# ucsdmanorlab/PSSR2

Hardware: AMD Instinct MI355X
Metric: HR tiles/sec (512^2 4xSR) train (higher is better)
Workload: dtype bf16

## Files before the change

include/pssr_mi355.h:

```cpp
#ifndef PSSR_MI355_H
#define PSSR_MI355_H

#include <stdint.h>

#ifdef __cplusplus
extern "C" {
#endif

typedef void* pssr_stream_t;

enum { PSSR_F32 = 0, PSSR_BF16 = 1, PSSR_F16 = 2 };

enum {
    PSSR_OK = 0,
    PSSR_ERR_ARG = -1,
    PSSR_ERR_LAUNCH = -2,
    PSSR_ERR_UNSUPPORTED = -3
};

int pssr_abi_version(void);
const char* pssr_last_error(void);

int pssr_pack_conv_weight(const float* w_oihw, void* packed, int cout, int cin, int ks,
                          int ci_begin, int ci_count, int mode, const int32_t* n_perm,
// ... 217 lines not shown
                         int dtype, pssr_stream_t stream);


int pssr_input_plain(const float* x_nchw, void* out, int n, int c, int h, int w, int out_cs, float pre_scale, float pre_shift,
                     int dtype, pssr_stream_t stream);
int pssr_im2col_dil(const void* in, int in_cs, int in_co, int c, const float* scale, const float* shift, void* col, int cp,
                    int n, int h, int w, int dil, int dtype, pssr_stream_t stream);
int pssr_col2im_dil(const void* dcol, int cp, void* out, int out_cs, int out_co, int c, int n, int h, int w, int dil,
                    const void* y, int y_cs, int y_co, const float* scale, const float* shift, const float* mean,
                    const float* invstd, double* stats, int dtype, pssr_stream_t stream);
int pssr_channel_stats_nhwc(const void* x, int cs, int co, int c, int64_t npix, double* stats, int dtype, pssr_stream_t stream);
int pssr_sum_relu(const void* const* ins, const int* in_cs, const int* in_co, int n_in, void* out, int out_cs, int out_co,
                  int64_t npix, int c, int relu, int dtype, pssr_stream_t stream);
int pssr_relu_mask(const void* dout, int do_cs, int do_co, const void* out, int o_cs, int o_co, void* dz, int dz_cs, int dz_co,
                   int64_t npix, int c, int dtype, pssr_stream_t stream);
int pssr_affine_relu(const void* x, int cs, int co, const float* scale, const float* shift, void* out, int out_cs, int out_co,
                     int64_t npix, int c, int dtype, pssr_stream_t stream);
int pssr_maxpool_k(const void* in, int in_cs, int in_co, void* out, int out_cs, int out_co, int n, int h, int w, int c, int k,
                   int dtype, pssr_stream_t stream);
int pssr_maxpool_k_bwd(const void* act, int act_cs, int act_co, const void* dpool, int dp_cs, int dp_co, void* dx, int dx_cs,
                       int dx_co, int n, int h, int w, int c, int k, int dtype, pssr_stream_t stream);
int pssr_bilinear_up(const void* in, int in_cs, int in_co, void* out, int out_cs, int out_co, int n, int hs, int ws, int h, int w,
                     int c, int dtype, pssr_stream_t stream);
int pssr_bilinear_up_bwd(const void* dout, int do_cs, int do_co, void* din, int di_cs, int di_co, int n, int hs, int ws, int h,
                         int w, int c, int dtype, pssr_stream_t stream);

int pssr_input_patchify(const float* x_nchw, void* xpatch, int n, int c, int h, int w, int ps, int pc,
                        float pre_scale, float pre_shift, const float* scale, const float* shift, int dtype,
                        pssr_stream_t stream);
int pssr_dwconv7_pack(const float* w, float* packed, int c, int flip, pssr_stream_t stream);
#define PSSR_DWPACK_BATCH_MAX 48
typedef struct pssr_dwpack_batch {
    const float* w[PSSR_DWPACK_BATCH_MAX];
    float* packed[PSSR_DWPACK_BATCH_MAX];
    int32_t c[PSSR_DWPACK_BATCH_MAX];
    int32_t flip[PSSR_DWPACK_BATCH_MAX];
} pssr_dwpack_batch;
int pssr_dwconv7_pack_batch(const pssr_dwpack_batch* items, int n_items, pssr_stream_t stream);
int pssr_dwconv7(const void* in, int in_cs, int in_co, const float* w_packed, const float* bias, void* out, int out_cs,
                 int out_co, int n, int h, int w, int c, int accumulate, int dtype, pssr_stream_t stream);
int pssr_dwconv7_wgrad(const void* dy, int dy_cs, int dy_co, const void* x, int x_cs, int x_co, float* dw, int n, int h,
                       int w, int c, int dtype, pssr_stream_t stream);
int64_t pssr_dwconv7_wgrad_workspace_bytes(int n, int h, int w, int c);
int pssr_dwconv7_wgrad_ws(const void* dy, int dy_cs, int dy_co, const void* x, int x_cs, int x_co, float* dw, int n, int h,
                          int w, int c, int dtype, void* workspace, int64_t workspace_bytes, pssr_stream_t stream);
int pssr_layernorm2d_fwd(const void* in, int in_cs, int in_co, const float* gamma, const float* beta, float eps, void* out,
                         int out_cs, int out_co, int s2d, int c_pad, int n, int h, int w, int c, float* mean, float* rstd,
                         int dtype, pssr_stream_t stream);
int pssr_layernorm2d_bwd(const void* g, int g_cs, int g_co, int s2d, int c_pad, const void* x, int x_cs, int x_co,
                         const float* gamma, const float* mean, const float* rstd, void* dx, int dx_cs, int dx_co,
                         int accumulate, int n, int h, int w, int c, double* stats, int dtype, pssr_stream_t stream);
int pssr_image_channel_dot(const void* a, int a_cs, int a_co, const void* b, int b_cs, int b_co, int n, int hw, int c,
                           float scale, float* out, int dtype, pssr_stream_t stream);
int64_t pssr_image_channel_dot_workspace_bytes(int n, int hw, int c);
int pssr_image_channel_dot_ws(const void* a, int a_cs, int a_co, const void* b, int b_cs, int b_co, int n, int hw, int c,
                              float scale, float* out, int dtype, void* workspace, int64_t workspace_bytes, pssr_stream_t stream);
int pssr_ese_gate(const float* s_mean, const float* w_fc, const float* b_fc, int n, int c, float* u, float* gate,
                  pssr_stream_t stream);
int pssr_scale_nc(const void* t, int t_cs, int t_co, const float* gate, const float* gamma, const float* add, void* out,
                  int out_cs, int out_co, int n, int hw, int c, int dtype, pssr_stream_t stream);
int pssr_ese_bwd(const float* A, const float* gate, const float* u, const float* gamma, const float* s_mean,
                 const float* w_fc, int n, int c, int hw, float* du, float* dgamma, float* db_fc, float* dw_fc, float* add,
                 pssr_stream_t stream);

int pssr_head_q_gather(const float* q, const float* bias, float* out_nchw, int n, int h, int w,
                       float out_scale, float out_shift, pssr_stream_t stream);

int pssr_head_conv_fwd(const void* act, int act_cs, int act_co, int blk, const float* w_oihw, const float* bias,
                       float* out_nchw, int n, int h, int w, int cin, int cout, float out_scale, float out_shift,
                       int dtype, pssr_stream_t stream);
int pssr_head_conv_dgrad(const float* g_nchw, float g_scale, const float* w_oihw, const void* act, int act_cs, int act_co,
                         void* dact, int d_cs, int d_co, int blk, int n, int h, int w, int cin, int cout, int dtype,
                         pssr_stream_t stream);
int pssr_head_conv_wgrad(const float* g_nchw, float g_scale, const void* act, int act_cs, int act_co, int blk,
                         float* dw_oihw, int n, int h, int w, int cin, int cout, int dtype, pssr_stream_t stream);
int pssr_head_conv_bwd(const float* g_nchw, float g_scale, const float* w_oihw, const void* act, int act_cs, int act_co,
                       void* dact, int d_cs, int d_co, int blk, float* dw_oihw, float* bias_sum, int n, int h, int w, int cin,
                       int cout, int dtype, pssr_stream_t stream);

int pssr_head_conv_bwd_rows(const float* g_nchw, float g_scale, const float* w_oihw, const void* act, int act_cs, int act_co,
                            void* dact, int d_cs, int d_co, int blk, double* dw_rows, double* bias_rows, int n, int h, int w,
                            int cin, int cout, int dtype, pssr_stream_t stream);

int pssr_sliding_tiles_u8(const uint8_t* sheet, float* tiles, int c, int h, int w, int size, int stride, int tile0, int ntile,
                          pssr_stream_t stream);
int pssr_patch_tiles_u8(const uint8_t* tiles, uint8_t* sheet, int c, int n_rows, int n_cols, int size, int overlap, int margin,
                        pssr_stream_t stream);


int64_t pssr_normalize_preds_workspace_bytes(int64_t pixels_per_image);
int pssr_normalize_preds_u8(const uint8_t* hr, const uint8_t* hr_hat, uint8_t* hr_norm, uint8_t* hr_hat_norm, int n_images,
                            int64_t pixels_per_image, float pmin, float pmax, void* workspace, pssr_stream_t stream);
int64_t pssr_normalize_preds_resized_workspace_bytes(int n_images, int H, int W, int h, int w);
int pssr_normalize_preds_resized_u8(const uint8_t* hr, int H, int W, const uint8_t* hr_hat, int h, int w, uint8_t* hr_norm,
                                    uint8_t* hr_hat_norm, int n_images, float pmin, float pmax, void* workspace,
                                    pssr_stream_t stream);

int64_t pssr_image_metrics_workspace_bytes(int n_images, int h, int w);
int pssr_image_metrics_u8(const uint8_t* hr, const uint8_t* hr_hat, double* out, int n_images, int h, int w, void* workspace,
                          pssr_stream_t stream);

#define PSSR_COPY_BATCH_MAX 16
typedef struct pssr_copy_batch {
    float* dst[PSSR_COPY_BATCH_MAX];
    const float* src[PSSR_COPY_BATCH_MAX];
    int64_t n[PSSR_COPY_BATCH_MAX];
} pssr_copy_batch;
int pssr_copy_f32_batch(const pssr_copy_batch* items, int n_items, pssr_stream_t stream);
typedef struct pssr_fold_batch {
    float* dst[PSSR_COPY_BATCH_MAX];
    const double* src[PSSR_COPY_BATCH_MAX];
    int32_t n[PSSR_COPY_BATCH_MAX];
    int32_t accumulate[PSSR_COPY_BATCH_MAX];
} pssr_fold_batch;
int pssr_f64_to_f32_batch(const pssr_fold_batch* items, int n_items, int stripes, pssr_stream_t stream);

#define PSSR_HIST_CLAMP 1
#define PSSR_HIST_ACCUMULATE 2
#define PSSR_HIST_MAX_BINS 8192
int64_t pssr_gradhist_workspace_bytes(int batch, int64_t n, int bins);
int pssr_gradhist_fwd(const float* a0, const float* b0, const float* a1, const float* b1, float* h0, float* h1, float* workspace,
                      int64_t workspace_bytes, int batch, int64_t n, int bins, float lo, float hi, float sigma, int flags,
                      pssr_stream_t stream);
int pssr_gradhist_bwd(const float* xa, const float* xb, const float* g, const float* g_ref, const float* dev_scale, float g_scale,
                      float* dx, int batch, int64_t n, int bins, float lo, float hi, float sigma, int flags, pssr_stream_t stream);
int pssr_crappifier_profiles(const float* lr_hat, const float* lr, const float* ds_hr, float* pred, float* target, int64_t n, int flags,
                             pssr_stream_t stream);
int pssr_subsample_f32(const float* src, float* dst, int64_t planes, int h_in, int w_in, int stride, pssr_stream_t stream);
int pssr_crappifier_loss_combine(const float* pred_hist, const float* target_hist, int64_t m, const float* ssim_loss, float dist_scale,
                                 float* out, pssr_stream_t stream);
int pssr_crappifier_loss_bwd_scalars(const float* parts, const float* grad_out, float* out, pssr_stream_t stream);
int pssr_clamp_f32(const float* x, float* y, int64_t n, float lo, float hi, pssr_stream_t stream);

#define PSSR_PROFILE_BINS 511
int64_t pssr_noise_profile_workspace_bytes(int images, int64_t per_image);
int pssr_noise_profile_f32(const float* a, const uint8_t* b, int32_t* hist, double* sum, int images, int64_t per_image, void* workspace,
                           int64_t workspace_bytes, pssr_stream_t stream);
int pssr_noise_profile_u8(const uint8_t* a, const uint8_t* b, int32_t* hist, double* sum, int images, int64_t per_image, void* workspace,
                          int64_t workspace_bytes, pssr_stream_t stream);
int pssr_noise_profile_loss(const int32_t* pred_hist, const double* pred_sum, const int32_t* target_hist, const double* target_sum,
                            int images, int64_t per_image, int width, double* loss, double* terms, double* mean, pssr_stream_t stream);

#ifdef __cplusplus
}
#endif
#endif
```

pssr2_amd/_lib.py:

```python
from __future__ import annotations

import ctypes as C
import os
from pathlib import Path

_LIB_PATH = Path(__file__).resolve().parent / "libpssr_mi355.so"
_lib = None

F32, BF16, F16 = 0, 1, 2
PRO_NONE, PRO_BN_RELU, PRO_GELU = 0, 1, 2
EPI_STORE, EPI_TAIL, EPI_DGRAD_MASK, EPI_FINAL, EPI_DGRAD_GELU, EPI_HEADQ = 0, 1, 2, 3, 4, 5
FLAG_RELU, FLAG_STATS, FLAG_AFFINE, FLAG_HEADQ, FLAG_SHUF2, FLAG_SOLO = 1, 2, 4, 8, 16, 32

c_void_p, c_int, c_i64, c_float = C.c_void_p, C.c_int, C.c_int64, C.c_float


class ConvDesc(C.Structure):
    _fields_ = [
        ("dtype", C.c_int32), ("n", C.c_int32), ("h", C.c_int32), ("w", C.c_int32),
        ("in0", c_void_p), ("in0_cstride", C.c_int32), ("in0_coff", C.c_int32), ("cin0", C.c_int32), ("taps0", C.c_int32),
        ("w0", c_void_p),
        ("in1", c_void_p), ("in1_cstride", C.c_int32), ("in1_coff", C.c_int32), ("cin1", C.c_int32), ("taps1", C.c_int32),
        ("w1", c_void_p),
        ("prologue", C.c_int32), ("pro_scale", c_void_p), ("pro_shift", c_void_p),
# ... 8 lines not shown
        ("workspace", c_void_p), ("workspace_bytes", C.c_int64),
        ("head_w", c_void_p), ("head_q", c_void_p),
    ]


class WgradDesc(C.Structure):
    _fields_ = [
        ("dtype", C.c_int32), ("n", C.c_int32), ("h", C.c_int32), ("w", C.c_int32),
        ("dy", c_void_p), ("dy_cstride", C.c_int32), ("dy_coff", C.c_int32), ("dy_blk", C.c_int32), ("cout", C.c_int32),
        ("in_", c_void_p), ("in_cstride", C.c_int32), ("in_coff", C.c_int32), ("in_blk", C.c_int32), ("cin_pad", C.c_int32),
        ("taps", C.c_int32),
        ("prologue", C.c_int32), ("pro_scale", c_void_p), ("pro_shift", c_void_p),
        ("dw", c_void_p), ("dw_parts", C.c_int32),
    ]


class GatherItem(C.Structure):
    _fields_ = [("src", C.c_void_p), ("sh", C.c_int), ("sw", C.c_int), ("rot", C.c_int), ("flip_axis", C.c_int)]


class SheetDesc(C.Structure):
    _fields_ = [("base", C.c_void_p), ("frames", C.c_int), ("h", C.c_int), ("w", C.c_int), ("reserved", C.c_int)]


class WindowItem(C.Structure):
    _fields_ = [("sheet", C.c_int), ("frame0", C.c_int), ("y0", C.c_int), ("x0", C.c_int), ("rot", C.c_int), ("flip_axis", C.c_int)]


class CollagePanel(C.Structure):
    _fields_ = [("src", C.c_void_p), ("image_stride", C.c_int64), ("row_pitch", C.c_int32), ("src_h", C.c_int32), ("src_w", C.c_int32),
                ("is_f32", C.c_int32), ("yi", C.c_void_p), ("xi", C.c_void_p)]


COPY_BATCH_MAX = 16


class FoldBatch(C.Structure):
    _fields_ = [("dst", C.c_void_p * 16), ("src", C.c_void_p * 16), ("n", C.c_int32 * 16), ("accumulate", C.c_int32 * 16)]


DWPACK_BATCH_MAX = 48


class DwPackBatch(C.Structure):
    _fields_ = [("w", C.c_void_p * DWPACK_BATCH_MAX), ("packed", C.c_void_p * DWPACK_BATCH_MAX), ("c", C.c_int32 * DWPACK_BATCH_MAX),
                ("flip", C.c_int32 * DWPACK_BATCH_MAX)]


class CopyBatch(C.Structure):
    _fields_ = [("dst", C.c_void_p * COPY_BATCH_MAX), ("src", C.c_void_p * COPY_BATCH_MAX), ("n", C.c_int64 * COPY_BATCH_MAX)]


class PackItem(C.Structure):
    _fields_ = [("w", c_void_p), ("packed", c_void_p), ("n_perm", c_void_p),
                ("cout", C.c_int32), ("cin", C.c_int32), ("ks", C.c_int32), ("ci_begin", C.c_int32), ("ci_count", C.c_int32),
                ("mode", C.c_int32), ("k_pad", C.c_int32), ("n_pad", C.c_int32), ("dtype", C.c_int32), ("center", C.c_int32)]


def lib():
    global _lib
    if _lib is None:
        if not _LIB_PATH.exists():
            raise RuntimeError(
                f"{_LIB_PATH} not found: build the HIP extension first (python -c 'import __graft_entry__ as g; g.build()' "
                "or make -C pssr2_amd/csrc). pssr2_amd has no CPU fallback.")
        import torch
        _lib = C.CDLL(str(_LIB_PATH))
        _lib.pssr_last_error.restype = C.c_char_p
        _lib.pssr_packed_weight_bytes.restype = C.c_int64
        _lib.pssr_conv2d_workspace_bytes.restype = C.c_int64
        _lib.pssr_gradhist_workspace_bytes.restype = C.c_int64
        _lib.pssr_noise_profile_workspace_bytes.restype = C.c_int64
        _lib.pssr_noise_profile_workspace_bytes.argtypes = [c_int, c_i64]
        for name in ("pssr_noise_profile_f32", "pssr_noise_profile_u8"):
            getattr(_lib, name).argtypes = [c_void_p, c_void_p, c_void_p, c_void_p, c_int, c_i64, c_void_p, c_i64, c_void_p]
        _lib.pssr_noise_profile_loss.argtypes = [c_void_p, c_void_p, c_void_p, c_void_p, c_int, c_i64, c_int, c_void_p, c_void_p, c_void_p,
                                                 c_void_p]
        _lib.pssr_gather_windows_u8.argtypes = [c_void_p, c_int, c_void_p, c_int, c_void_p, c_int, c_int, c_void_p]
        _lib.pssr_collage_rows_u8.argtypes = [c_void_p, c_int, c_void_p, c_i64, c_int, c_int, c_int, c_int, c_void_p]
        _lib.pssr_window_attn_workspace_bytes.restype = c_i64
        _lib.pssr_window_attn_workspace_bytes.argtypes = [c_int] * 5
        _lib.pssr_window_attn_fwd.argtypes = [c_void_p] * 4 + [c_int] * 7 + [c_float, c_int, c_void_p]
        _lib.pssr_window_attn_bwd.argtypes = [c_void_p] * 7 + [c_i64] + [c_int] * 7 + [c_float, c_int, c_void_p]
    return _lib


def check(status: int, what: str):
    if status != 0:
        raise RuntimeError(f"{what} failed ({status}): {lib().pssr_last_error().decode()}")


def ptr(t):
    return None if t is None else c_void_p(t.data_ptr())


def stream_ptr():
    import torch
    return c_void_p(torch.cuda.current_stream().cuda_stream)
```

pssr2_amd/engine.py:

```python
from __future__ import annotations

import os
from types import SimpleNamespace

import torch

from . import _lib as L
from . import atrous as A
from . import ops

BN_EPS, BN_MOMENTUM = 1e-5, 0.1


def _blocked_order(r: int):
    if r < 1:
        raise ValueError(f"upscaling factor must be a positive integer, got scale={r}")
    l = r.bit_length() - 1
    return (l, False) if (1 << l) == r else (0, True)


_NO_MATERIALISE = os.environ.get("PSSR_MATERIALISE", "0") != "1"
_XCOL_SIDE = os.environ.get("PSSR_XCOL_SIDE", "0") == "1"
_FUSE_DOUT = os.environ.get("PSSR_FUSE_DOUT", "1") != "0"
_OVERWRITE_GRADS = os.environ.get("PSSR_OVERWRITE_GRADS", "1") != "0"
_EVAL_SHUF = os.environ.get("PSSR_EVAL_SHUF", "1") != "0"
_EVAL_AFFINE = os.environ.get("PSSR_EVAL_AFFINE", "1") != "0"
_HEAD_FUSE = os.environ.get("PSSR_HEAD_FUSE", "1") != "0"

FWD, DGRAD = dict(mode=0), dict(mode=1)
FWD_FLAT, DGRAD_FLAT = dict(mode=2), dict(mode=3)
FWD_CENTER, DGRAD_CENTER = dict(mode=2, center=True), dict(mode=3, center=True)


class _Arena:

    def __init__(self):
        self.req = []

    def take(self, n):
        self.req.append(n)
        return len(self.req) - 1

    def build(self, dtype, device):
        offs, tot = [], 0
        for n in self.req:
            offs.append(tot)
            tot += (n + 3) // 4 * 4
        self.buf = torch.zeros(max(tot, 4), dtype=dtype, device=device)
        self.views = [self.buf[o:o + n] for o, n in zip(offs, self.req)]
        return self


class _BNState:
    def __init__(self, c, f32: _Arena, f64: _Arena):
        self.c = c
        self.i32 = [f32.take(c) for _ in range(7)]
        self.i64 = [f64.take(2 * c * ops.STAT_STRIPES) for _ in range(2)]

    def bind(self, f32: _Arena, f64: _Arena):
        self.scale, self.shift, self.mean, self.invstd, self.ca, self.cb, self.cc = (f32.views[i] for i in self.i32)
        self.stats, self.bstats = (f64.views[i] for i in self.i64)
        self.eval_key = None


class _Conv:

    def __init__(self, module, specs, wepoch=None):
        self.m = module
        self.specs = specs
        self.packed = {}
        self.version = {}
        self.wepoch = wepoch if wepoch is not None else [0]

    def ver(self):
        return (self.wepoch[0], self.m.weight._version)

    def weight_for(self, spec):
        w = self.m.weight
        if spec.get("center"):
            w3 = torch.zeros(w.shape[0], w.shape[1], 3, 3, device=w.device, dtype=w.dtype)
            w3[:, :, 1, 1] = w.detach()[:, :, 0, 0]
            return w3
        return w.detach()

    def item(self, name, dtype):
        spec, pw, w = self.specs[name], self.packed[(name, dtype)], self.m.weight
        center = bool(spec.get("center"))
        it = L.PackItem()
        it.w, it.packed = w.data_ptr(), pw.data.data_ptr()
        perm = spec.get("n_perm")
        it.n_perm = perm.data_ptr() if perm is not None else None
        it.cout, it.cin, it.ks = w.shape[0], w.shape[1], 3 if center else w.shape[2]
        it.ci_begin = spec.get("ci_begin", 0)
        it.ci_count = spec.get("ci_count") if spec.get("ci_count") is not None else w.shape[1] - it.ci_begin
        it.mode, it.k_pad, it.n_pad, it.dtype, it.center = spec["mode"], pw.k_pad, pw.n_pad, dtype, int(center)
        return it

    def get(self, name, dtype):
        spec = self.specs[name]
        key = (name, dtype)
        ver = self.ver()
        if self.version.get(key) != ver or key not in self.packed:
            self.packed[key] = ops.pack_conv_weight(self.weight_for(spec).contiguous(), dtype, mode=spec["mode"],
                                                    ci_begin=spec.get("ci_begin", 0), ci_count=spec.get("ci_count"),
                                                    n_perm=spec.get("n_perm"), out=self.packed.get(key))
            self.version[key] = ver
# ... 616 lines not shown
        ops.conv2d(feat, h0, pw0, p.pre, r * r * h0, n=n, h=h, w=w, bias=p.pre_bias, x1=p.xcol, cin1=self.xc, w1=pw1, flags=L.FLAG_RELU)
        pre_hr = self._pre_hr(p)
        if self.explicit_shuffle:
            ops.pixel_shuffle(p.pre, pre_hr, n, h, w, h0, r, code)
        if ops.head_conv_supported(code, h0, self.cout):
            ops.head_conv_fwd(pre_hr, self.blk, rec.conv.weight, rec.conv.bias, out, n, h * r, w * r, h0, self.cout, 128.0, 128.0, code)
        else:
            ops.conv2d(pre_hr, h0, self._pw(rec.conv, "fwd", code, **FWD), out, self.cout, n=n, h=h * r, w=w * r, bias=rec.conv.bias,
                       epilogue=L.EPI_FINAL, in0_blk=self.blk, out_scale=128.0, out_shift=128.0)
        return out

    def _pw_pre(self, name, code):
        return self._pw(self.model.reconstruction.pre, name, code, **self.pre_specs[name])

    def _rows_head(self, code):
        return ops.head_conv_supported(code, self.h0, self.cout) and not self.explicit_shuffle and self.blk <= 2 and self.h0 in (32, 64, 128)

    def _pre_hr(self, p):
        n, h, w, r, h0 = p.n, p.h, p.w, self.r, self.h0
        if not self.explicit_shuffle:
            return p.pre.view(n, h * r, w * r, h0)
        if p.pre_hr is None:
            p.pre_hr = torch.zeros(n, h * r, w * r, h0, dtype=p.pre.dtype, device=p.pre.device)
        return p.pre_hr

    def _head_backward(self, p, bw, grads, dout, feat, dfeat):
        rec = self.model.reconstruction
        n, h, w, code, h0, r = p.n, p.h, p.w, p.code, self.h0, self.r
        dev = dout.device
        H, W = h * r, w * r
        dout = dout.contiguous().float()
        pre_hr = self._pre_hr(p)
        if self.explicit_shuffle:
            if bw.dpre_hr is None:
                bw.dpre_hr = torch.zeros_like(pre_hr)
            dpre_hr = bw.dpre_hr
        else:
            dpre_hr = bw.dpre.view(n, H, W, h0)
        if ops.head_conv_supported(code, h0, self.cout):
            gw = grads[id(rec.conv.weight)] = self._gbuf(rec.conv.weight)
            gb = torch.empty(2 * self.cout, dtype=torch.float32, device=dev)
            grads[id(rec.conv.bias)] = gb[:self.cout]
            gpb = torch.empty(r * r * h0, dtype=torch.float32, device=dev) if self._rows_head(code) else None
            if gpb is not None:
                S = ops.STAT_STRIPES
                sizes = (S * 2 * self.cout, S * gw.numel(), S * gpb.numel())
                if bw.h64 is None or bw.h64.numel() != sum(sizes):
                    bw.h64 = torch.zeros(sum(sizes), dtype=torch.float64, device=dev)
                else:
                    bw.h64.zero_()
                s_out, dw64, s_pre = torch.split(bw.h64, sizes)
                ops.channel_stats_nchw(dout, s_out, 128.0, 0.0)
                ops.head_conv_bwd_rows(dout, 128.0, rec.conv.weight, pre_hr, dpre_hr, self.blk, dw64, s_pre, n, H, W, h0, self.cout, code)
                ops.f64_to_f32_batch([(s_out, gb, False), (dw64, gw.view(-1), False), (s_pre, gpb, False)])
            else:
                bw.sum64.zero_()
                ops.channel_stats_nchw(dout, bw.sum64, 128.0, 0.0)
                ops.f64_to_f32(bw.sum64[:ops.STAT_STRIPES * 2 * self.cout], gb)
                ops.head_conv_wgrad(dout, 128.0, pre_hr, self.blk, gw, n, H, W, h0, self.cout, code)
                ops.head_conv_dgrad(dout, 128.0, rec.conv.weight, pre_hr, dpre_hr, self.blk, n, H, W, h0, self.cout, code)
        else:
            gpb = None
            ops.nchw_to_nhwc(dout, bw.g_hr, 128.0, code)
            bw.sum64.zero_()
            ops.channel_sum_nhwc(bw.g_hr, n * H * W, 16, bw.sum64, code)
            gb = torch.empty(16, dtype=torch.float32, device=dev)
            ops.f64_to_f32(bw.sum64, gb)
            grads[id(rec.conv.bias)] = gb[:self.cout]
            self._wgrad(p, grads, rec.conv, bw.g_hr, 16, pre_hr, h0, 9, in_blk=self.blk, hh=H, ww=W)
            ops.conv2d(bw.g_hr, 16, self._pw(rec.conv, "dgrad", code, **DGRAD), dpre_hr, h0, n=n, h=H, w=W, epilogue=L.EPI_DGRAD_MASK,
                       aux=pre_hr, aux_scale=p.ones_pre, aux_shift=p.zeros_pre, out_blk=self.blk, aux_blk=self.blk)
        cpre_n = r * r * h0
        if self.explicit_shuffle:
            ops.pixel_shuffle(bw.dpre, dpre_hr, n, h, w, h0, r, code, inverse=True)
        if gpb is None:
            bw.sum64.zero_()
            ops.channel_sum_nhwc(bw.dpre, n * h * w, cpre_n, bw.sum64, code)
            gpb = torch.empty(cpre_n, dtype=torch.float32, device=dev)
            ops.f64_to_f32(bw.sum64, gpb)
        gb_pre = torch.empty_like(gpb)
        gb_pre[self.pre_perm_long] = gpb
        grads[id(rec.pre.bias)] = gb_pre
        self._wgrad(p, grads, rec.pre, bw.dpre, cpre_n, feat, h0, 9, mode=0, ci_begin=0, ci_count=h0, n_perm=self.pre_perm, hh=h, ww=w)
        self._wgrad(p, grads, rec.pre, bw.dpre, cpre_n, p.xcol, self.xc, 1, mode=2, ci_begin=h0, ci_count=self.cin, n_perm=self.pre_perm, hh=h, ww=w)
        self._ready(grads, list(rec.parameters()))
        ops.conv2d(bw.dpre, cpre_n, self._pw_pre("dgrad0", code), dfeat, h0, n=n, h=h, w=w)
        if not self.atrous:
            pw1 = self._pw_pre("dgrad1", code)

            def dgrad_x():
                ops.conv2d(bw.dpre, cpre_n, pw1, bw.dxcol_b, self.xc, n=n, h=h, w=w)
            if self._side_on and _XCOL_SIDE:
                self._on_side([bw.dpre, bw.dxcol_b], dgrad_x)
            else:
                dgrad_x()

    @staticmethod
    def _wgrad_rows(cout, code):
        esz = 4 if code == L.F32 else 2
        return cout if (cout * esz) % 16 == 0 else ops.pad_to(cout, 16)

    def _wgrad1x1(self, grads, conv_module, dy, cout, dy_coff, src, cin_pad, n, hh, ww, code, *, side, mode=0, pro=None, src_coff=0,
                  gelu_in=False, first=None):
        rows = self._wgrad_rows(cout, code)
        assert rows == cout or dy_coff == 0
        slot = grads[id(conv_module.weight)] = self._gbuf(conv_module.weight)

        def run():
            if first is not None:
                first()
            parts = ops.conv2d_wgrad_parts(dy, rows, src, cin_pad, 1, n=n, h=hh, w=ww, dtype=code, dy_coff=dy_coff, in_coff=src_coff, gelu_in=gelu_in,
                                           pro_scale=pro.scale if pro is not None else None, pro_shift=pro.shift if pro is not None else None)
            ops.unpack_conv_wgrad(parts, slot, mode=mode, k_pad=cin_pad, accumulate=True)
        if side and self._side_on:
            self._on_side([dy], run)
        else:
            run()

    def _wgrad(self, p, grads, conv_module, dy, cout, src, cin_pad, taps, *, mode=0, ci_begin=0, ci_count=None,
               n_perm=None, pro=None, dy_blk=0, in_blk=0, hh, ww, center=False, dy_view_c=None):
        code = p.code
        co_eff = self._wgrad_rows(cout, code)
        w = conv_module.weight
        gname = id(w)

        def parts():
            return ops.conv2d_wgrad_parts(dy, co_eff, src, cin_pad, taps, n=p.n, h=hh, w=ww, dtype=code, dy_blk=dy_blk, in_blk=in_blk,
                                          pro_scale=pro.scale if pro else None, pro_shift=pro.shift if pro else None)
        if center:
            g3 = torch.zeros(w.shape[0], w.shape[1], 3, 3, dtype=torch.float32, device=w.device)
            ops.unpack_conv_wgrad(parts(), g3, mode=mode, ci_begin=ci_begin, ci_count=ci_count, n_perm=n_perm, k_pad=cin_pad)
            grads[gname] = g3[:, :, 1:2, 1:2].contiguous()
            return
        if gname not in grads:
            grads[gname] = self._gbuf(w)
        slot = grads[gname]

        def run():
            ops.unpack_conv_wgrad(parts(), slot, mode=mode, ci_begin=ci_begin, ci_count=ci_count, n_perm=n_perm, k_pad=cin_pad,
                                  accumulate=not self._overwrite_grads)
        if self._side_on:
            self._on_side([dy], run)
        else:
            run()

    def _fused_dout(self, p, blk, kind):
        if blk.a is not None or not _FUSE_DOUT:
            return False
        return ops.relu_bwd_stats_fused_ok(p.code, blk.c, *p.dims[blk.level], unshuffle=kind == "unshuffle")

    def _block_backward(self, p, bw, grads, blk, module, src, cin, first, out_buf, out_coff, dout, dsrc, dsrc_c, dout_from=None):
        if blk.a is not None:
            A.ablock_backward(self, blk.a, module, grads, p.xin if first else src, 0, p.n, p.code, out_buf, out_coff, dout, 0, dsrc, not first)
            return
        n, code = p.n, p.code
        lvl = blk.level
        hh, ww = p.dims[lvl]
        npix = n * hh * ww
        count = float(npix)
        nl = len(blk.y)
        dz, g = bw.dz[lvl], bw.g[lvl]
        ring = [bw.dy[lvl], bw.dy2[lvl], bw.dy3[lvl]] if self._side_on else [bw.dy[lvl]]
        ri = 0
        dy = ring[0]
        last = blk.bn[-1]
        bn_last = module.conv[3 * (nl - 1) + 1]
        self._before_write(dz)
        if dout_from is None:
            ops.relu_bwd_stats(dout, out_buf, blk.y[-1], last.mean, last.invstd, dz, last.bstats, npix, blk.c, code, out_coff=out_coff)
        elif dout_from[0] == "pool":
# ... 113 lines not shown
```

pssr2_amd/ops.py:

```python
from __future__ import annotations

import ctypes as C

import torch

from . import _lib as L

TORCH_DTYPE = {L.F32: torch.float32, L.BF16: torch.bfloat16, L.F16: torch.float16}


def dtype_code(dt: torch.dtype) -> int:
    if dt == torch.float32:
        return L.F32
    if dt == torch.bfloat16:
        return L.BF16
    if dt == torch.float16:
        return L.F16
    raise ValueError(f"unsupported compute dtype {dt}; use torch.float32, torch.bfloat16 or torch.float16")


def pad_to(v: int, m: int) -> int:
    return (v + m - 1) // m * m


# ... 414 lines not shown
                    accumulate=False):
    c_pad = pad_to(c, 16) if c_pad is None else c_pad
    L.check(L.lib().pssr_layernorm2d_bwd(*_ref(g, g_coff), int(s2d), c_pad, *_ref(x, x_coff), L.ptr(gamma), L.ptr(mean), L.ptr(rstd),
                                         *_ref(dx, dx_coff), int(accumulate), n, h, w, c, L.ptr(stats), dtype, L.stream_ptr()),
            "pssr_layernorm2d_bwd")


def image_channel_dot(a, b, n, hw, c, scale, out, dtype, a_coff=0, b_coff=0):
    bref = _ref(b, b_coff) if b is not None else (None, 0, 0)
    L.check(L.lib().pssr_image_channel_dot(*_ref(a, a_coff), *bref, n, hw, c, C.c_float(scale), L.ptr(out), dtype, L.stream_ptr()),
            "pssr_image_channel_dot")


def ese_gate(s_mean, w_fc, b_fc, u, gate):
    n, c = s_mean.shape
    L.check(L.lib().pssr_ese_gate(L.ptr(s_mean), L.ptr(w_fc), L.ptr(b_fc), n, c, L.ptr(u), L.ptr(gate), L.stream_ptr()), "pssr_ese_gate")


def scale_nc(t, gate, gamma, add, out, n, hw, c, dtype, t_coff=0, out_coff=0):
    L.check(L.lib().pssr_scale_nc(*_ref(t, t_coff), L.ptr(gate), L.ptr(gamma), L.ptr(add), *_ref(out, out_coff), n, hw, c, dtype,
                                  L.stream_ptr()), "pssr_scale_nc")


def ese_bwd(A, gate, u, gamma, s_mean, w_fc, hw, du, dgamma, db_fc, dw_fc, add):
    n, c = A.shape
    L.check(L.lib().pssr_ese_bwd(L.ptr(A), L.ptr(gate), L.ptr(u), L.ptr(gamma), L.ptr(s_mean), L.ptr(w_fc), n, c, hw, L.ptr(du),
                                 L.ptr(dgamma), L.ptr(db_fc), L.ptr(dw_fc), L.ptr(add), L.stream_ptr()), "pssr_ese_bwd")


def head_conv_supported(dtype, cin, cout):
    return dtype in (L.BF16, L.F16) and 1 <= cout <= 3 and cin % 32 == 0 and 32 <= cin <= 128


def head_conv_fwd(act, blk, weight, bias, out, n, h, w, cin, cout, out_scale, out_shift, dtype, act_coff=0):
    L.check(L.lib().pssr_head_conv_fwd(L.ptr(act), act.shape[-1], act_coff, blk, L.ptr(weight), L.ptr(bias), L.ptr(out), n, h, w, cin, cout,
                                       C.c_float(out_scale), C.c_float(out_shift), dtype, L.stream_ptr()), "pssr_head_conv_fwd")


def head_conv_dgrad(g, g_scale, weight, act, dact, blk, n, h, w, cin, cout, dtype, *, act_coff=0, dact_coff=0):
    L.check(L.lib().pssr_head_conv_dgrad(L.ptr(g), C.c_float(g_scale), L.ptr(weight), L.ptr(act), act.shape[-1], act_coff, L.ptr(dact), dact.shape[-1], dact_coff,
                                         blk, n, h, w, cin, cout, dtype, L.stream_ptr()), "pssr_head_conv_dgrad")


def head_conv_wgrad(g, g_scale, act, blk, dw, n, h, w, cin, cout, dtype, *, act_coff=0):
    L.check(L.lib().pssr_head_conv_wgrad(L.ptr(g), C.c_float(g_scale), L.ptr(act), act.shape[-1], act_coff, blk, L.ptr(dw), n, h, w, cin, cout, dtype,
                                         L.stream_ptr()), "pssr_head_conv_wgrad")


def sliding_tiles_u8(sheet, size, stride, tile0, ntile):
    c, h, w = sheet.shape
    out = torch.empty(ntile, c, size, size, dtype=torch.float32, device=sheet.device)
    L.check(L.lib().pssr_sliding_tiles_u8(L.ptr(sheet), L.ptr(out), c, h, w, size, stride, tile0, ntile, L.stream_ptr()), "pssr_sliding_tiles_u8")
    return out


def patch_tiles_u8(tiles, n_rows, n_cols, overlap, margin):
    t, c, size, _ = tiles.shape
    assert t == n_rows * n_cols and tiles.dtype == torch.uint8 and tiles.is_contiguous()
    step = size - overlap
    out = torch.empty(c, n_rows * step + overlap, n_cols * step + overlap, dtype=torch.uint8, device=tiles.device)
    L.check(L.lib().pssr_patch_tiles_u8(L.ptr(tiles), L.ptr(out), c, n_rows, n_cols, size, overlap, margin, L.stream_ptr()), "pssr_patch_tiles_u8")
    return out


def head_conv_bwd(g, g_scale, weight, act, dact, blk, dw, bias_sum, n, h, w, cin, cout, dtype, *, act_coff=0, dact_coff=0):
    L.check(L.lib().pssr_head_conv_bwd(L.ptr(g), C.c_float(g_scale), L.ptr(weight), L.ptr(act), act.shape[-1], act_coff, L.ptr(dact), dact.shape[-1], dact_coff,
                                       blk, L.ptr(dw), L.ptr(bias_sum), n, h, w, cin, cout, dtype, L.stream_ptr()), "pssr_head_conv_bwd")


def head_q_supported(dtype, h0, cout, r, h, w):
    return dtype != L.F32 and h0 == 64 and cout == 1 and r == 4 and h >= 16 and w >= 16 and L.lib().pssr_get_option(b"IGEMM_V3") > 0


def head_q_gather(q, bias, out, n, h, w, out_scale, out_shift):
    L.check(L.lib().pssr_head_q_gather(L.ptr(q), L.ptr(bias), L.ptr(out), n, h, w, C.c_float(out_scale), C.c_float(out_shift), L.stream_ptr()),
            "pssr_head_q_gather")


def head_conv_bwd_rows(g, g_scale, weight, act, dact, blk, dw_rows, bias_rows, n, h, w, cin, cout, dtype, *, act_coff=0, dact_coff=0):
    L.check(L.lib().pssr_head_conv_bwd_rows(L.ptr(g), C.c_float(g_scale), L.ptr(weight), L.ptr(act), act.shape[-1], act_coff, L.ptr(dact), dact.shape[-1], dact_coff,
                                            blk, L.ptr(dw_rows), L.ptr(bias_rows), n, h, w, cin, cout, dtype, L.stream_ptr()), "pssr_head_conv_bwd_rows")


def crappify_saltpepper(x, amount, gain, spread, seed, tile_offset, flags, out=None, tile_counter=None):
    out = torch.empty_like(x) if out is None else out
    tiles = x.shape[0]
    L.check(L.lib().pssr_crappify_saltpepper(L.ptr(x), L.ptr(out), tiles, C.c_int64(x.numel() // tiles), C.c_float(amount), C.c_float(gain),
                                             C.c_float(spread), C.c_uint64(seed), C.c_uint64(tile_offset), flags, L.ptr(tile_counter),
                                             L.stream_ptr()), "pssr_crappify_saltpepper")
    return out


def gaussian_blur_tiles(x, sigma, spread, gain, seed, tile_offset, flags, tile_counter=None):
    tiles, h, w = x.shape[0], x.shape[-2], x.shape[-1]
    tmp, out = torch.empty_like(x), torch.empty_like(x)
    L.check(L.lib().pssr_gaussian_blur_tiles(L.ptr(x), L.ptr(tmp), L.ptr(out), tiles, x.numel() // (tiles * h * w), h, w, C.c_float(sigma),
                                             C.c_float(spread), C.c_float(gain), C.c_uint64(seed), C.c_uint64(tile_offset), flags,
                                             L.ptr(tile_counter), L.stream_ptr()), "pssr_gaussian_blur_tiles")
    return out


def gen_pair_geometry_u8(stacks, rotations, res):
    c = stacks[0].shape[0]
    items = (L.GatherItem * len(stacks))()
    for i, (st, rot) in enumerate(zip(stacks, rotations)):
        if st.dtype != torch.uint8 or not st.is_cuda or st.dim() != 3 or st.shape[0] != c or not st.is_contiguous():
            raise ValueError("gen_pair_geometry_u8 needs contiguous uint8 [c, h, w] stacks on the device")
        axis = -1
        if rot:
            axis = 3 if isinstance(rot[1], (tuple, list)) else int(rot[1])
        items[i].src, items[i].sh, items[i].sw = st.data_ptr(), st.shape[1], st.shape[2]
        items[i].rot, items[i].flip_axis = int(bool(rot and rot[0])), axis
    table = torch.frombuffer(bytearray(bytes(items)), dtype=torch.uint8).to(stacks[0].device)
    out = torch.empty(len(stacks), c, res, res, dtype=torch.uint8, device=stacks[0].device)
    L.check(L.lib().pssr_gen_pair_geometry_u8(L.ptr(table), len(stacks), L.ptr(out), c, res, L.stream_ptr()), "pssr_gen_pair_geometry_u8")
    return out


def gather_windows_u8(sheet_table, n_sheets, items, c, res):
    for t, size in ((sheet_table, n_sheets), (items, None)):
        if not t.is_cuda or not t.is_contiguous() or (t.numel() * t.element_size()) % 24 or (size is not None and t.numel() * t.element_size() != 24 * size):
            raise ValueError("gather_windows_u8 needs contiguous device tables of 24-byte records")
    n = items.numel() * items.element_size() // 24
    out = torch.empty(n, c, res, res, dtype=torch.uint8, device=items.device)
    L.check(L.lib().pssr_gather_windows_u8(L.ptr(sheet_table), n_sheets, L.ptr(items), n, L.ptr(out), c, res, L.stream_ptr()), "pssr_gather_windows_u8")
    return out


def nearest_index(src, dst):
    import numpy as np
    if src < 1 or dst < 1:
        raise ValueError(f"nearest_index needs positive sizes, got {src} -> {dst}")
    a = float(src) / float(dst)
    xo, out = 0.5 * a, np.empty(dst, dtype=np.int32)
    for x in range(dst):
        out[x] = int(xo)
        xo += a
    return out


_NEAREST_TABLES = {}


def nearest_table(src, dst, device):
    key = (int(src), int(dst), str(torch.device(device)))
    t = _NEAREST_TABLES.get(key)
    if t is None:
        t = _NEAREST_TABLES[key] = torch.from_numpy(nearest_index(int(src), int(dst))).to(device)
    return t


def collage_rows_u8(panels, canvas, row0=0):
    if not 1 <= len(panels) <= 3:
        raise ValueError("collage_rows_u8 takes 1 to 3 panels")
    if canvas.dtype != torch.uint8 or not canvas.is_cuda or canvas.dim() != 2 or canvas.stride(1) != 1:
        raise ValueError("collage_rows_u8 needs a uint8 device canvas [rows, columns] with unit column stride")
    descs, keep, size, n = (L.CollagePanel * len(panels))(), [], None, None
    for d, panel in zip(descs, panels):
        src, yi, xi = panel if isinstance(panel, (tuple, list)) else (panel, None, None)
        if src.dtype not in (torch.uint8, torch.float32) or src.dim() != 3 or src.device != canvas.device or min(src.shape) < 1:
            raise ValueError("collage_rows_u8: a panel source is a non-empty uint8 or float32 tensor [n, h, w] on the canvas's device")
        if src.stride(2) != 1 or src.stride(1) < src.shape[2] or src.stride(0) < 0:
            src = src.contiguous()
        if (yi is None) != (xi is None):
            raise ValueError("collage_rows_u8: a panel has one index table but not the other")
        for t in (yi, xi):
# ... 278 lines not shown
```

Baseline: 2386.

## Fuse xcol weight-grad and data-grad into one paired backward kernel

Adds a HIP kernel that reads the pre-conv output gradient once per pixel tile and computes both the 1x1 weight gradient against the xcol input and the data gradient into dxcol. Per-block partial weight slabs are then summed by a small reduction kernel. This replaces a separate wgrad call and a separate dgrad conv, so dy, the large-channel tensor, is read once instead of twice. In exchange it adds a slab reduction pass and an unpack step, and it only applies to 16-bit dtypes, kx=16 and cout a multiple of 64.

```diff
diff --git a/include/pssr_mi355.h b/include/pssr_mi355.h
--- a/include/pssr_mi355.h
+++ b/include/pssr_mi355.h
@@ -323,6 +323,12 @@
                             void* dact, int d_cs, int d_co, int blk, double* dw_rows, double* bias_rows, int n, int h, int w,
                             int cin, int cout, int dtype, pssr_stream_t stream);
 
+int pssr_flatk_bwd_pair_supported(int dtype, int cout, int kx);
+int pssr_flatk_bwd_pair_parts(int64_t npix);
+int pssr_flatk_bwd_pair(const void* dy, int dy_cs, int dy_co, int cout, const void* x, int x_cs, int x_co, void* dx, int dx_cs,
+                        int dx_co, int kx, const float* w, int w_row, int w_off, int nk, const int32_t* n_perm, float* slabs,
+                        int parts, float* dw, int64_t npix, int dtype, pssr_stream_t stream);
+
 int pssr_sliding_tiles_u8(const uint8_t* sheet, float* tiles, int c, int h, int w, int size, int stride, int tile0, int ntile,
                           pssr_stream_t stream);
 int pssr_patch_tiles_u8(const uint8_t* tiles, uint8_t* sheet, int c, int n_rows, int n_cols, int size, int overlap, int margin,
diff --git a/pssr2_amd/_lib.py b/pssr2_amd/_lib.py
--- a/pssr2_amd/_lib.py
+++ b/pssr2_amd/_lib.py
@@ -114,6 +114,10 @@
         _lib.pssr_window_attn_workspace_bytes.argtypes = [c_int] * 5
         _lib.pssr_window_attn_fwd.argtypes = [c_void_p] * 4 + [c_int] * 7 + [c_float, c_int, c_void_p]
         _lib.pssr_window_attn_bwd.argtypes = [c_void_p] * 7 + [c_i64] + [c_int] * 7 + [c_float, c_int, c_void_p]
+        _lib.pssr_flatk_bwd_pair_supported.argtypes = [c_int] * 3
+        _lib.pssr_flatk_bwd_pair_parts.argtypes = [c_i64]
+        _lib.pssr_flatk_bwd_pair.argtypes = ([c_void_p] + [c_int] * 3 + [c_void_p] + [c_int] * 2 + [c_void_p] + [c_int] * 3 + [c_void_p] + [c_int] * 3
+                                             + [c_void_p] * 2 + [c_int, c_void_p, c_i64, c_int, c_void_p])
     return _lib
 
 
diff --git a/pssr2_amd/csrc/pre_xcol_bwd.hip b/pssr2_amd/csrc/pre_xcol_bwd.hip
--- /dev/null
+++ b/pssr2_amd/csrc/pre_xcol_bwd.hip
@@ -0,0 +1,268 @@
+
+#include "common.h"
+
+namespace {
+
+constexpr int PX_PIX = 64;
+constexpr int PX_CH = 256;
+constexpr int PX_KX = 16;
+constexpr int PX_ROWB = 64;
+constexpr int PX_SUB = PX_PIX * PX_ROWB;
+constexpr int PX_DY_BYTES = (PX_CH / 32) * PX_SUB;
+constexpr int PX_XT_BYTES = PX_PIX * PX_ROWB;
+constexpr int PX_DX_BYTES = 2 * PX_PIX * PX_KX * 4;
+constexpr int PX_ITEMS = PX_DY_BYTES / 16 / 256;
+constexpr int PX_RED_LANES = 16;
+
+struct PairArgs {
+    const void* dy; int dy_cs, dy_co, cout;
+    const void* x; int x_cs, x_co;
+    void* dx; int dx_cs, dx_co;
+    const float* w; int w_row, w_off, nk;
+    const int32_t* n_perm;
+    float* slabs;
+    long npix; int n_tiles;
+};
+
+template <typename T> constexpr int px_w1_stride(int nch) { return (nch * PX_CH + 8) * (int)sizeof(T); }
+template <typename T> constexpr int px_lds_bytes(int nch) { return PX_DY_BYTES + PX_XT_BYTES + PX_DX_BYTES + PX_KX * px_w1_stride<T>(nch); }
+
+__device__ __forceinline__ u32x4 px_tr_frag(const char* a0, const char* a1) {
+    typedef __attribute__((ext_vector_type(4))) short s16x4;
+    typedef __attribute__((ext_vector_type(2))) unsigned int u32x2;
+    const u32x2 lo = __builtin_bit_cast(u32x2, __builtin_amdgcn_ds_read_tr16_b64_v4i16((__attribute__((address_space(3))) s16x4*)a0));
+    const u32x2 hi = __builtin_bit_cast(u32x2, __builtin_amdgcn_ds_read_tr16_b64_v4i16((__attribute__((address_space(3))) s16x4*)a1));
+    u32x4 r = {lo[0], lo[1], hi[0], hi[1]};
+    return r;
+}
+
+template <typename T, int NCH>
+__global__ __launch_bounds__(256, 2) void flatk_bwd_pair_kernel(const PairArgs p) {
+    using X = TT<T>;
+    constexpr int ESZ = 2;
+    constexpr int W1S = px_w1_stride<T>(NCH);
+    static_assert(sizeof(T) == 2, "16-bit storage");
+    extern __shared__ __attribute__((aligned(16))) char smem[];
+    char* const Dy = smem;
+    char* const Xt = smem + PX_DY_BYTES;
+    float* const Dxs = (float*)(smem + PX_DY_BYTES + PX_XT_BYTES);
+    char* const W1t = smem + PX_DY_BYTES + PX_XT_BYTES + PX_DX_BYTES;
+
+    const int tid = threadIdx.x, lane = tid & 63, wave = tid >> 6;
+    const int t_begin = (int)((long)blockIdx.x * p.n_tiles / gridDim.x), t_end = (int)((long)(blockIdx.x + 1) * p.n_tiles / gridDim.x);
+
+    for (int i = tid; i < NCH * PX_CH * PX_KX; i += 256) {
+        const int k = i / PX_KX, j = i % PX_KX;
+        float v = 0.f;
+        if (k < p.cout && j < p.nk) v = p.w[(long)(p.n_perm ? p.n_perm[k] : k) * p.w_row + p.w_off + j];
+        *(T*)(W1t + j * W1S + k * ESZ) = (T)v;
+    }
+    if (tid < 2 * PX_PIX) *(u32x4*)(Xt + (tid >> 1) * PX_ROWB + 32 + (tid & 1) * 16) = u32x4{0u, 0u, 0u, 0u};
+
+    f32x16 accw[NCH][2];
+#pragma unroll
+    for (int c = 0; c < NCH; ++c)
+#pragma unroll
+        for (int a = 0; a < 2; ++a)
+#pragma unroll
+            for (int e = 0; e < 16; ++e) accw[c][a][e] = 0.f;
+
+    const int ipix = tid >> 3, ipc = tid & 7;
+    const unsigned dy_off0 = (unsigned)((ipix * p.dy_cs + ipc * 8) * ESZ), dy_off1 = dy_off0 + (unsigned)(32 * p.dy_cs * ESZ);
+    const int dy_lds = (ipc >> 2) * PX_SUB + ipix * PX_ROWB + (ipc & 3) * 16;
+    const unsigned x_off = (unsigned)(((tid >> 1) * p.x_cs + (tid & 1) * 8) * ESZ);
+    const int x_lds = (tid >> 1) * PX_ROWB + (tid & 1) * 16;
+    const int g = lane >> 4, li = lane & 15;
+    const int fr_off = ((g >> 1) * 8 + (li >> 2)) * PX_ROWB + ((g & 1) * 16 + (li & 3) * 4) * 2;
+    const char* const dyw_rd = Dy + (2 * wave) * PX_SUB + fr_off;
+    const char* const x_rd = Xt + fr_off;
+    const int mblk = wave & 1, kgrp = wave >> 1;
+    const char* const dyd_rd = Dy + (kgrp * 4) * PX_SUB + (mblk * 32 + (lane & 31)) * PX_ROWB + (lane >> 5) * 16;
+    const char* const w1_rd = W1t + (lane & 15) * W1S + (kgrp * 128 + (lane >> 5) * 8) * ESZ;
+
+    u32x4 dy_reg[PX_ITEMS], x_reg = {0u, 0u, 0u, 0u};
+
+#define PX_ISSUE(TILE, CH)                                                                                        \
+    {                                                                                                             \
+        const long pix0_ = (long)(TILE) * PX_PIX;                                                                 \
+        const int left_ = (int)(p.npix - pix0_ < PX_PIX ? p.npix - pix0_ : PX_PIX);                               \
+        const __amdgpu_buffer_rsrc_t rdy_ = __builtin_amdgcn_make_buffer_rsrc(                                    \
+            (void*)((const char*)p.dy + (pix0_ * p.dy_cs + p.dy_co + (CH) * PX_CH) * ESZ), 0, (int)0xfffffff0u, 0x00020000); \
+        _Pragma("unroll") for (int it = 0; it < PX_ITEMS; ++it) {                                                 \
+            const bool ok_ = ipix + 32 * (it & 1) < left_ && (CH) * PX_CH + 64 * (it >> 1) < p.cout;              \
+            const unsigned off_ = ok_ ? ((it & 1) ? dy_off1 : dy_off0) + (unsigned)(128 * (it >> 1)) : 0xffffffffu; \
+            dy_reg[it] = __builtin_bit_cast(u32x4, __builtin_amdgcn_raw_buffer_load_b128(rdy_, (int)off_, 0, 0)); \
+        }                                                                                                         \
+        if ((CH) == 0 && tid < 128) {                                                                             \
+            const __amdgpu_buffer_rsrc_t rx_ = __builtin_amdgcn_make_buffer_rsrc(                                 \
+                (void*)((const char*)p.x + (pix0_ * p.x_cs + p.x_co) * ESZ), 0, (int)0xfffffff0u, 0x00020000);    \
+            x_reg = __builtin_bit_cast(u32x4, __builtin_amdgcn_raw_buffer_load_b128(rx_, (int)((tid >> 1) < left_ ? x_off : 0xffffffffu), 0, 0)); \
+        }                                                                                                         \
+    }
+
+    if (t_begin < t_end) PX_ISSUE(t_begin, 0)
+    for (int tile = t_begin; tile < t_end; ++tile) {
+        f32x16 accd;
+#pragma unroll
+        for (int e = 0; e < 16; ++e) accd[e] = 0.f;
+#pragma unroll
+        for (int c = 0; c < NCH; ++c) {
+#pragma unroll
+            for (int it = 0; it < PX_ITEMS; ++it) *(u32x4*)(Dy + dy_lds + (it >> 1) * 2 * PX_SUB + (it & 1) * 32 * PX_ROWB) = dy_reg[it];
+            if (c == 0 && tid < 128) *(u32x4*)(Xt + x_lds) = x_reg;
+            __syncthreads();
+            if (c + 1 < NCH) PX_ISSUE(tile, c + 1)
+            else if (tile + 1 < t_end) PX_ISSUE(tile + 1, 0)
+
+#pragma unroll
+            for (int s = 0; s < PX_PIX / 16; ++s) {
+                const u32x4 bf = px_tr_frag(x_rd + s * 16 * PX_ROWB, x_rd + (s * 16 + 4) * PX_ROWB);
+#pragma unroll
+                for (int a = 0; a < 2; ++a) {
+                    const u32x4 af = px_tr_frag(dyw_rd + a * PX_SUB + s * 16 * PX_ROWB, dyw_rd + a * PX_SUB + (s * 16 + 4) * PX_ROWB);
+                    X::mma(accw[c][a], af, bf);
+                }
+            }
+#pragma unroll
+            for (int ss = 0; ss < 4; ++ss)
+#pragma unroll
+                for (int t = 0; t < 2; ++t) {
+                    const u32x4 af = *(const u32x4*)(dyd_rd + ss * PX_SUB + t * 32);
+                    const u32x4 bf = *(const u32x4*)(w1_rd + (c * PX_CH + ss * 32 + t * 16) * ESZ);
+                    X::mma(accd, af, bf);
+                }
+            __syncthreads();
+        }
+        if ((lane & 31) < PX_KX) {
+#pragma unroll
+            for (int e = 0; e < 16; ++e) {
+                const int row = mblk * 32 + (e & 3) + 8 * (e >> 2) + 4 * (lane >> 5);
+                Dxs[(kgrp * PX_PIX + row) * PX_KX + (lane & 31)] = accd[e];
+            }
+        }
+        __syncthreads();
+        {
+            const int row = tid >> 2, j0 = (tid & 3) * 4;
+            const long pix = (long)tile * PX_PIX + row;
+            if (pix < p.npix) {
+                const float4 a = *(const float4*)(Dxs + row * PX_KX + j0);
+                const float4 b = *(const float4*)(Dxs + (PX_PIX + row) * PX_KX + j0);
+                const float v[4] = {a.x + b.x, a.y + b.y, a.z + b.z, a.w + b.w};
+                store4((T*)p.dx + pix * p.dx_cs + p.dx_co + j0, v);
+            }
+        }
+    }
+#undef PX_ISSUE
+
+    if ((lane & 31) < PX_KX) {
+        float* const dst = p.slabs + (long)blockIdx.x * p.cout * PX_KX;
+#pragma unroll
+        for (int c = 0; c < NCH; ++c)
+#pragma unroll
+            for (int a = 0; a < 2; ++a)
+#pragma unroll
+                for (int e = 0; e < 16; ++e) {
+                    const int n = c * PX_CH + (2 * wave + a) * 32 + (e & 3) + 8 * (e >> 2) + 4 * (lane >> 5);
+                    if (n < p.cout) dst[n * PX_KX + (lane & 31)] = accw[c][a][e];
+                }
+    }
+}
+
+__global__ __launch_bounds__(256) void flatk_slab_sum_kernel(const float* __restrict__ slabs, int parts, int total4, float* __restrict__ dw) {
+    __shared__ float4 buf[256];
+    const int pos = threadIdx.x & 15, pl = threadIdx.x >> 4;
+    const int i4 = blockIdx.x * 16 + pos;
+    float4 v = make_float4(0.f, 0.f, 0.f, 0.f);
+    if (i4 < total4)
+        for (int q = pl; q < parts; q += PX_RED_LANES) {
+            const float4 a = *(const float4*)(slabs + ((long)q * total4 + i4) * 4);
+            v.x += a.x; v.y += a.y; v.z += a.z; v.w += a.w;
+        }
+    buf[pl * 16 + pos] = v;
+    __syncthreads();
+    if (pl == 0 && i4 < total4) {
+        float4 s = buf[pos];
+        for (int l = 1; l < PX_RED_LANES; ++l) {
+            const float4 a = buf[l * 16 + pos];
+            s.x += a.x; s.y += a.y; s.z += a.z; s.w += a.w;
+        }
+        *(float4*)(dw + (long)i4 * 4) = s;
+    }
+}
+
+int px_cus() {
+    static int cus = 0;
+    if (cus == 0) {
+        int dev = 0, n = 0;
+        if (hipGetDevice(&dev) == hipSuccess && hipDeviceGetAttribute(&n, hipDeviceAttributeMultiprocessorCount, dev) == hipSuccess && n > 0) cus = n;
+        else cus = 256;
+    }
+    return cus;
+}
+
+int px_parts(long npix) {
+    const long tiles = (npix + PX_PIX - 1) / PX_PIX;
+    const long target = 2L * px_cus();
+    return (int)(tiles < target ? tiles : target);
+}
+
+template <typename T, int NCH>
+int px_launch(const PairArgs& a, int parts, hipStream_t s) {
+    constexpr int LDS = px_lds_bytes<T>(NCH);
+    static_assert(2 * LDS <= 160 * 1024, "two workgroups per CU");
+    static bool attr_done = false;
+    if (!attr_done) {
+        (void)hipFuncSetAttribute((const void*)flatk_bwd_pair_kernel<T, NCH>, hipFuncAttributeMaxDynamicSharedMemorySize, LDS);
+        attr_done = true;
+    }
+    hipLaunchKernelGGL((flatk_bwd_pair_kernel<T, NCH>), dim3(parts), dim3(256), LDS, s, a);
+    PSSR_LAUNCH_CHECK();
+    return PSSR_OK;
+}
+
+template <typename T>
+int px_launch_nch(const PairArgs& a, int parts, hipStream_t s) {
+    const int nch = cdiv(a.cout, PX_CH);
+    return nch == 1 ? px_launch<T, 1>(a, parts, s) : nch == 2 ? px_launch<T, 2>(a, parts, s)
+         : nch == 3 ? px_launch<T, 3>(a, parts, s) : px_launch<T, 4>(a, parts, s);
+}
+
+}
+
+extern "C" int pssr_flatk_bwd_pair_supported(int dtype, int cout, int kx) {
+    return (dtype == PSSR_BF16 || dtype == PSSR_F16) && cout >= 64 && cout <= 4 * PX_CH && cout % 64 == 0 && kx == PX_KX;
+}
+
+extern "C" int pssr_flatk_bwd_pair_parts(int64_t npix) {
+    PSSR_CHECK(npix > 0 && npix < (1LL << 31) * PX_PIX, PSSR_ERR_ARG, "flatk_bwd_pair: npix=%lld", (long long)npix);
+    return px_parts((long)npix);
+}
+
+extern "C" int pssr_flatk_bwd_pair(const void* dy, int dy_cs, int dy_co, int cout, const void* x, int x_cs, int x_co, void* dx, int dx_cs,
+                                   int dx_co, int kx, const float* w, int w_row, int w_off, int nk, const int32_t* n_perm, float* slabs,
+                                   int parts, float* dw, int64_t npix, int dtype, pssr_stream_t stream) {
+    PSSR_CHECK(dy && x && dx && w && slabs && dw, PSSR_ERR_ARG, "flatk_bwd_pair: null pointer");
+    PSSR_CHECK(pssr_flatk_bwd_pair_supported(dtype, cout, kx), PSSR_ERR_UNSUPPORTED,
+               "flatk_bwd_pair: dtype=%d cout=%d kx=%d (16-bit storage, cout a multiple of 64 up to 1024, kx = 16)", dtype, cout, kx);
+    PSSR_CHECK(npix > 0 && npix < (1LL << 31) * PX_PIX, PSSR_ERR_ARG, "flatk_bwd_pair: npix=%lld", (long long)npix);
+    PSSR_CHECK(dy_cs % 8 == 0 && dy_co % 8 == 0 && dy_co >= 0 && dy_co + cout <= dy_cs, PSSR_ERR_ARG, "flatk_bwd_pair: dy stride/offset");
+    PSSR_CHECK(x_cs % 8 == 0 && x_co % 8 == 0 && x_co >= 0 && x_co + kx <= x_cs, PSSR_ERR_ARG, "flatk_bwd_pair: x stride/offset");
+    PSSR_CHECK(dx_cs % 4 == 0 && dx_co % 4 == 0 && dx_co >= 0 && dx_co + kx <= dx_cs, PSSR_ERR_ARG, "flatk_bwd_pair: dx stride/offset");
+    PSSR_CHECK((long)PX_PIX * dy_cs * 2 < (1L << 30) && (long)PX_PIX * x_cs * 2 < (1L << 30), PSSR_ERR_ARG, "flatk_bwd_pair: channel stride too large");
+    PSSR_CHECK(nk > 0 && nk <= kx && w_row >= w_off + nk && w_off >= 0, PSSR_ERR_ARG, "flatk_bwd_pair: weight window");
+    PSSR_CHECK(parts == px_parts((long)npix), PSSR_ERR_ARG, "flatk_bwd_pair: parts=%d but this shape needs %d (ask pssr_flatk_bwd_pair_parts)", parts,
+               px_parts((long)npix));
+    PairArgs a;
+    a.dy = dy; a.dy_cs = dy_cs; a.dy_co = dy_co; a.cout = cout;
+    a.x = x; a.x_cs = x_cs; a.x_co = x_co;
+    a.dx = dx; a.dx_cs = dx_cs; a.dx_co = dx_co;
+    a.w = w; a.w_row = w_row; a.w_off = w_off; a.nk = nk; a.n_perm = n_perm;
+    a.slabs = slabs; a.npix = (long)npix; a.n_tiles = (int)((npix + PX_PIX - 1) / PX_PIX);
+    hipStream_t s = (hipStream_t)stream;
+    const int rc = dtype == PSSR_BF16 ? px_launch_nch<bf16_t>(a, parts, s) : px_launch_nch<f16_t>(a, parts, s);
+    if (rc != PSSR_OK) return rc;
+    const int total4 = cout * PX_KX / 4;
+    hipLaunchKernelGGL(flatk_slab_sum_kernel, dim3(cdiv(total4, 16)), dim3(256), 0, s, (const float*)slabs, parts, total4, dw);
+    PSSR_LAUNCH_CHECK();
+    return PSSR_OK;
+}
diff --git a/pssr2_amd/engine.py b/pssr2_amd/engine.py
--- a/pssr2_amd/engine.py
+++ b/pssr2_amd/engine.py
@@ -22,6 +22,7 @@
 _NO_MATERIALISE = os.environ.get("PSSR_MATERIALISE", "0") != "1"
 _XCOL_SIDE = os.environ.get("PSSR_XCOL_SIDE", "0") == "1"
 _FUSE_DOUT = os.environ.get("PSSR_FUSE_DOUT", "1") != "0"
+_XCOL_FUSE = os.environ.get("PSSR_XCOL_FUSE", "1") != "0"
 _OVERWRITE_GRADS = os.environ.get("PSSR_OVERWRITE_GRADS", "1") != "0"
 _EVAL_SHUF = os.environ.get("PSSR_EVAL_SHUF", "1") != "0"
 _EVAL_AFFINE = os.environ.get("PSSR_EVAL_AFFINE", "1") != "0"
@@ -804,10 +805,23 @@
         gb_pre[self.pre_perm_long] = gpb
         grads[id(rec.pre.bias)] = gb_pre
         self._wgrad(p, grads, rec.pre, bw.dpre, cpre_n, feat, h0, 9, mode=0, ci_begin=0, ci_count=h0, n_perm=self.pre_perm, hh=h, ww=w)
-        self._wgrad(p, grads, rec.pre, bw.dpre, cpre_n, p.xcol, self.xc, 1, mode=2, ci_begin=h0, ci_count=self.cin, n_perm=self.pre_perm, hh=h, ww=w)
+        fuse_x = _XCOL_FUSE and not self.atrous and not self.explicit_shuffle and ops.flatk_bwd_pair_supported(code, cpre_n, self.xc)
+        if fuse_x:
+            slot = grads[id(rec.pre.weight)]
+
+            def pair_x():
+                dw1 = ops.flatk_bwd_pair(bw.dpre, cpre_n, p.xcol, bw.dxcol_b, rec.pre.weight, code, ci_begin=h0, ci_count=self.cin, n_perm=self.pre_perm)
+                ops.unpack_conv_wgrad(dw1, slot, mode=2, ci_begin=h0, ci_count=self.cin, n_perm=self.pre_perm, k_pad=self.xc,
+                                      accumulate=not self._overwrite_grads)
+            if self._side_on:
+                self._on_side([bw.dpre, p.xcol, bw.dxcol_b], pair_x)
+            else:
+                pair_x()
+        else:
+            self._wgrad(p, grads, rec.pre, bw.dpre, cpre_n, p.xcol, self.xc, 1, mode=2, ci_begin=h0, ci_count=self.cin, n_perm=self.pre_perm, hh=h, ww=w)
         self._ready(grads, list(rec.parameters()))
         ops.conv2d(bw.dpre, cpre_n, self._pw_pre("dgrad0", code), dfeat, h0, n=n, h=h, w=w)
-        if not self.atrous:
+        if not self.atrous and not fuse_x:
             pw1 = self._pw_pre("dgrad1", code)
 
             def dgrad_x():
diff --git a/pssr2_amd/ops.py b/pssr2_amd/ops.py
--- a/pssr2_amd/ops.py
+++ b/pssr2_amd/ops.py
@@ -520,6 +520,27 @@
                                             blk, L.ptr(dw_rows), L.ptr(bias_rows), n, h, w, cin, cout, dtype, L.stream_ptr()), "pssr_head_conv_bwd_rows")
 
 
+def flatk_bwd_pair_supported(dtype, cout, kx):
+    return bool(L.lib().pssr_flatk_bwd_pair_supported(dtype, cout, kx))
+
+
+def flatk_bwd_pair(dy, cout, x, dx, weight, dtype, *, ci_begin, ci_count, n_perm=None, dy_coff=0):
+    kx = x.shape[-1]
+    npix = dy.numel() // dy.shape[-1]
+    assert x.numel() // kx == npix and dx.numel() // dx.shape[-1] == npix and dx.shape[-1] == kx
+    assert weight.dtype == torch.float32 and weight.is_contiguous() and weight.dim() == 4
+    kk = weight.shape[2] * weight.shape[3]
+    parts = L.lib().pssr_flatk_bwd_pair_parts(npix)
+    if parts <= 0:
+        L.check(parts if parts < 0 else -1, "pssr_flatk_bwd_pair_parts")
+    slabs = torch.empty(parts, cout, kx, dtype=torch.float32, device=dy.device)
+    dw = torch.empty(1, cout, 1, kx, dtype=torch.float32, device=dy.device)
+    L.check(L.lib().pssr_flatk_bwd_pair(L.ptr(dy), dy.shape[-1], dy_coff, cout, L.ptr(x), kx, 0, L.ptr(dx), kx, 0, kx, L.ptr(weight),
+                                        weight.shape[1] * kk, ci_begin * kk, ci_count * kk, L.ptr(n_perm), L.ptr(slabs), parts, L.ptr(dw), npix, dtype,
+                                        L.stream_ptr()), "pssr_flatk_bwd_pair")
+    return dw
+
+
 def crappify_saltpepper(x, amount, gain, spread, seed, tile_offset, flags, out=None, tile_counter=None):
     out = torch.empty_like(x) if out is None else out
     tiles = x.shape[0]
```

Measured after the change: 2426, median of 6. 1.7% higher.
